# SJLeo/GCC

Measured on AMD Instinct MI355X. Metric: training images/sec at 256x256 (pix2pix GCC), higher is better.
Workload: dtype bf16; 1 GPU; Pix2Pix cityscapes 256x256 GCC distill+darts iteration (optimize_parameters + optimizer_netD_arch), student ngf32 / masked PatchGAN ndf128, teacher ngf64 / ndf128, filter_cfgs=None (no pretrained checkpoint to prune); batch_per_gpu=16, global_batch=16, image=256x256, parallelism=dp1, dropout=on (counter RNG; the oracle / golden iterations run --no_dropout)

## Files before the change

gcc_amd/csrc/conv_igemm.hip:

```cpp
#include <stdlib.h>
#include <mutex>
#include "common.hpp"
#include "igemm_common.hpp"

#ifndef GCC_IGEMM_ROT
#define GCC_IGEMM_ROT 0
#endif

namespace gcc_igemm {

#ifdef GCC_CLOCK_PROBE
__device__ unsigned long long g_clock_probe[4096][8];
#endif

template <int BP, int BC, bool UT, int NS = 2, bool EV = false>
__global__ __launch_bounds__((BP / 32) * 64) void igemm_kernel(const IgemmArgs<EV> p) {
    constexpr int EPI = EV ? 1 : 0;
#include "igemm_kernel_body.inc"
}

template <int BP, int BC, bool UT, int NS = 2>
__global__ __launch_bounds__((BP / 32) * 64) void igemm_ex_kernel(const IgemmExParams p) {
    constexpr int EPI = 2;
#include "igemm_kernel_body.inc"
// ... 375 lines not shown
    else if (Cout > 32) { t.BC = 64; t.ntiles = 1; }
    else if (Cout > 16) { t.BC = 32; t.ntiles = 1; }
    else { t.BC = 16; t.ntiles = 1; }
    if (batch == 1 && t.BC > 32) {
        const long mt = (long)((max_rows + 127) / 128) * phases;
        if (nk <= 64) {
            int bc = t.BC;
            while (bc > 32 && mt * cdiv(Cout, bc) < 256) bc >>= 1;
            if (mt * cdiv(Cout, bc) >= 256) { t.BC = bc; t.ntiles = cdiv(Cout, bc); }
        } else if (mt >= 8 && mt * cdiv(Cout, t.BC) < 128) {
            t.BC = 64; t.ntiles = cdiv(Cout, 64); t.max_slices = 8;
        }
    }
    const int g_big_tiles = plan_or(pl.tile_families, PLAN_TILE_FAMILIES) - 1, g_big_min = plan_or(pl.big_min, PLAN_BIG_MIN),
              g_big_nk = plan_or(pl.big_nk, PLAN_BIG_NK);
    if (g_big_tiles && batch == 1 && Cout >= 128 && nk >= g_big_nk) {
        const long m256 = (long)((max_rows + 255) / 256);
        if (g_big_tiles >= 2 && Cout % 256 == 0 && m256 * (Cout / 256) * phases >= g_big_min) {
            t.BP = 256; t.BC = 256; t.ntiles = Cout / 256;
            t.pair = (pl.pair == 1 && m256 * (Cout / 256) * phases < 192 && nk >= 48) ? 1 : 0;
        } else if (m256 * cdiv(Cout, 128) * phases >= g_big_min) {
            t.BP = 256; t.BC = 128; t.ntiles = cdiv(Cout, 128);
        }
    }
    t.mtiles = (int)((max_rows + t.BP - 1) / t.BP);
    return t;
}
constexpr size_t PAIR_FLAG_BYTES = 4096;
static size_t pair_workspace(size_t tiles) { return tiles > 512 ? ~(size_t)0 : PAIR_FLAG_BYTES + tiles * (size_t)(256 * 256 * 4); }
static int conv_nk(const gcc_conv_t* c, int dgrad) {
    const int taps_max = dgrad ? cdiv(c->KH, c->stride) * cdiv(c->KW, c->stride) : c->KH * c->KW;
    return cdiv(taps_max * ceil8(dgrad ? c->Co : c->Ci), BK);
}
static size_t conv_max_rows(const gcc_conv_t* c, int dgrad) {
    if (!dgrad) return (size_t)c->N * gcc_conv_out(c->H, c->KH, c->stride, c->pad) * gcc_conv_out(c->W, c->KW, c->stride, c->pad);
    return (size_t)c->N * cdiv(c->H, c->stride) * cdiv(c->W, c->stride);
}

int check_conv(const gcc_conv_t* c) {
    if (!c) return GCC_ERR_BAD_ARG;
    if (c->N <= 0 || c->H <= 0 || c->W <= 0 || c->Ci <= 0 || c->Co <= 0 || c->KH <= 0 || c->KW <= 0 ||
        c->stride <= 0 || c->pad < 0)
        return GCC_ERR_BAD_ARG;
    if ((c->ldx & 7) || (c->xoff & 7) || (c->ldy & 7) || (c->yoff & 7)) return GCC_ERR_BAD_ARG;
    if (c->ldx < c->xoff + ceil8(c->Ci) || c->ldy < c->yoff + ceil8(c->Co)) return GCC_ERR_BAD_ARG;
    if (gcc_conv_out(c->H, c->KH, c->stride, c->pad) <= 0 || gcc_conv_out(c->W, c->KW, c->stride, c->pad) <= 0)
        return GCC_ERR_BAD_ARG;
    return GCC_OK;
}

}
using namespace gcc_igemm;

struct HeadArgs {
    const float* partial; int ksplit, rows_max, Cpad;
    const float* bias; int act; float slope;
    bf16_t* dst; int ldd, doff;
    const bf16_t* dy; int lddy, dyoff;
    bf16_t* g;
    int N, H, W, Ho, Wo, KH, KW, stride, pad;
};
__global__ __launch_bounds__(256) void head_tapsum_kernel(const HeadArgs a) {
    const size_t total = (size_t)a.N * a.Ho * a.Wo;
    const int tap = threadIdx.x & 15;
    const int kh = tap / a.KW, kw = tap - kh * a.KW;
    for (size_t q0 = (size_t)blockIdx.x * 16; q0 < total; q0 += (size_t)gridDim.x * 16) {
        const size_t q = q0 + (threadIdx.x >> 4);
        float acc = 0.f;
        if (q < total && kh < a.KH) {
            const int ox = (int)(q % a.Wo);
            const size_t t = q / a.Wo;
            const int oy = (int)(t % a.Ho);
            const size_t n = t / a.Ho;
            const int iy = oy * a.stride + kh - a.pad, ix = ox * a.stride + kw - a.pad;
            if ((unsigned)iy < (unsigned)a.H && (unsigned)ix < (unsigned)a.W) {
                const size_t row = (n * a.H + iy) * (size_t)a.W + ix;
                for (int s = 0; s < a.ksplit; s++) acc += a.partial[((size_t)s * a.rows_max + row) * a.Cpad + tap];
            }
        }
#pragma unroll
        for (int o = 8; o > 0; o >>= 1) acc += __shfl_xor(acc, o, 16);
        if (tap == 0 && q < total) {
            float o[8] = {0, 0, 0, 0, 0, 0, 0, 0};
            o[0] = apply_act(acc + (a.bias ? a.bias[0] : 0.f), a.act, a.slope);
            *(i32x4*)(a.dst + q * a.ldd + a.doff) = pack8(o);
        }
    }
}
__global__ __launch_bounds__(256) void head_gather_kernel(const HeadArgs a) {
    const int taps = a.KH * a.KW;
    const size_t total = (size_t)a.N * a.H * a.W * taps;
    for (size_t q = (size_t)blockIdx.x * 256 + threadIdx.x; q < total; q += (size_t)gridDim.x * 256) {
        const int tap = (int)(q % taps);
        const size_t pix = q / taps;
        const int ix = (int)(pix % a.W);
        const size_t t = pix / a.W;
        const int iy = (int)(t % a.H);
        const size_t n = t / a.H;
        const int kh = tap / a.KW, kw = tap - kh * a.KW;
        const int ny = iy + a.pad - kh, nx = ix + a.pad - kw;
        float o[8] = {0, 0, 0, 0, 0, 0, 0, 0};
        if (ny >= 0 && nx >= 0 && ny % a.stride == 0 && nx % a.stride == 0) {
            const int oy = ny / a.stride, ox = nx / a.stride;
            if (oy < a.Ho && ox < a.Wo) o[0] = bf2f(a.dy[((n * a.Ho + oy) * (size_t)a.Wo + ox) * a.lddy + a.dyoff]);
        }
        *(i32x4*)(a.g + q * 8) = pack8(o);
// ... 429 lines not shown
        std::call_once(wide_once, [] {
            (void)hipFuncSetAttribute((const void*)thin_dgrad_wide_kernel, hipFuncAttributeMaxDynamicSharedMemorySize, 156 * 1024);
        });
        int wpi = 256 / c->N;
        if (wpi < 1) wpi = 1;
        if (wpi > a.Ho) wpi = a.Ho;
        const int rows_per_wg = cdiv(a.Ho, wpi);
        wpi = cdiv(a.Ho, rows_per_wg);
        hipLaunchKernelGGL(thin_dgrad_wide_kernel, dim3(c->N * wpi), dim3(THIN_WIDE_NT), lds, st, a, rows_per_wg, wpi);
        GCC_CHECK_LAUNCH();
        return GCC_OK;
    }
    const int ncc = a.Co8 > 32 ? 2 : 1;
    int wgs = cdiv(a.ntiles, 4);
    if (wgs > 768) wgs = 768;
    const dim3 grid(wgs, 2);
    if (ncc == 2) hipLaunchKernelGGL(thin_dgrad_k4s2_kernel<2>, grid, dim3(256), 0, st, a);
    else hipLaunchKernelGGL(thin_dgrad_k4s2_kernel<1>, grid, dim3(256), 0, st, a);
    GCC_CHECK_LAUNCH();
    return GCC_OK;
}

extern "C" int gcc_conv_y2_supported(const gcc_conv_t* c, int dgrad, const gcc_epilogue_t* ep) {
    if (check_conv(c) || dgrad || !ep || !thin_shape(c)) return 0;
    if (ep->stats_partial || ep->act == GCC_ACT_TANH || (ep->act == GCC_ACT_LRELU && (ep->slope < 0.f || ep->slope > 1.f))) return 0;
    if ((ep->ldy2 & 7) || (ep->y2off & 7)) return 0;
    if (ep->y2_mode == 1) return ep->act == GCC_ACT_LRELU || ep->act == GCC_ACT_NONE;
    if (ep->y2_mode == 2) return ep->y2_gate != nullptr;
    return 0;
}

int gcc_internal_thinout_fprop(const gcc_conv_t* c, const void* x, const void* w, void* y, const gcc_epilogue_t* ep, hipStream_t st);
int gcc_internal_thinout_dgrad(const gcc_conv_t* c, const void* dy, const void* wt, void* dx, const gcc_epilogue_t* ep, hipStream_t st);
int gcc_internal_ring3(const gcc_conv_t* c, int dgrad, const void* src, const void* w, void* dst, const gcc_epilogue_t* ep, hipStream_t st);
int gcc_internal_ring3_rows(const gcc_conv_t* c, int dgrad);
bool gcc_internal_ring3_routed(const gcc_conv_t* c, int dgrad, const gcc_epilogue_t* ep);

constexpr size_t FUSE_BN_PARTIAL_BYTES = (size_t)4096 * 1024;

int gcc_internal_igemm(const gcc_conv_t* c, int dgrad, const void* src, const void* w, void* dst, const gcc_epilogue_t* ep,
                       int batch, long src_bstride, long wgt_bstride, long dst_bstride, hipStream_t st) {
    GCC_ENTER();
    int rc = check_conv(c);
    if (rc) return rc;
    if (!src || !w || !dst) return GCC_ERR_BAD_ARG;
    const int Ho = gcc_conv_out(c->H, c->KH, c->stride, c->pad);
    const int Wo = gcc_conv_out(c->W, c->KW, c->stride, c->pad);
    if (batch == 1 && head_shape(c) && ep && ep->workspace && !ep->stats_partial && (((uintptr_t)ep->workspace) & 15) == 0) {
        const int taps = c->KH * c->KW;
        if (!dgrad) {
            int ks = 1;
            const size_t need = head_fprop_workspace(c, &ks);
            if (need <= ep->workspace_bytes) {
                IgemmParams q;
                q.src = (const bf16_t*)src; q.wgt = (const bf16_t*)w; q.dst = (bf16_t*)dst; q.bias = nullptr; q.stats = nullptr;
                q.act = GCC_ACT_NONE; q.slope = 0.f;
                q.N = c->N; q.KH = 1; q.KW = 1; q.stride = 1; q.pad = 0; q.dgrad = 0;
                q.Hs = c->H; q.Ws = c->W; q.lds_ = c->ldx; q.soff = c->xoff; q.Hd = c->H; q.Wd = c->W; q.ldd = c->ldy; q.doff = c->yoff;
                q.Ct = ceil8(c->Ci); q.Cout = taps; q.ldw = q.Ct;
                const size_t rows = head_rows(c);
                const size_t sb = rows * (size_t)q.lds_ * 2, wb = (size_t)taps * q.ldw * 2;
                if (sb < OOB && wb < OOB) {
                    q.src_bytes = (uint32_t)sb; q.wgt_bytes = (uint32_t)wb;
                    q.src_bstride = q.wgt_bstride = q.dst_bstride = 0;
                    q.ntiles = 1; q.mtiles_max = cdiv((int)rows, 128);
                    const int nk = cdiv(q.Ct, BK);
                    q.ksplit = ks; q.kper = cdiv(nk, ks); q.partial = (float*)ep->workspace; q.rows_max = (int)rows; q.Cpad = 16;
                    q.raw_partial = 1;
                    int rc2 = launch<128, 16>(q, 1, 1, st);
                    if (rc2) return rc2;
                    HeadArgs a = {};
                    a.partial = q.partial; a.ksplit = q.ksplit; a.rows_max = q.rows_max; a.Cpad = 16;
                    a.bias = ep->bias; a.act = ep->act; a.slope = ep->slope;
                    a.dst = (bf16_t*)dst; a.ldd = c->ldy; a.doff = c->yoff;
                    a.N = c->N; a.H = c->H; a.W = c->W; a.Ho = Ho; a.Wo = Wo; a.KH = c->KH; a.KW = c->KW; a.stride = c->stride; a.pad = c->pad;
                    const size_t outs = (size_t)c->N * Ho * Wo;
                    hipLaunchKernelGGL(head_tapsum_kernel, dim3((unsigned)(outs + 15 > 16 * 4096 ? 4096 : (outs + 15) / 16)), dim3(256), 0, st, a);
                    GCC_CHECK_LAUNCH();
                    return GCC_OK;
                }
            }
        }
    }
    if (batch == 1 && dgrad && thin_dgrad_shape(c) && !(ep && ep->stats_partial)) {
        const int rc2 = launch_thin_dgrad(c, src, w, dst, ep, st);
        if (rc2 >= 0) return rc2;
    }
    if (batch == 1) {
        const int rc3 = dgrad ? gcc_internal_thinout_dgrad(c, src, w, dst, ep, st) : gcc_internal_thinout_fprop(c, src, w, dst, ep, st);
        if (rc3 != GCC_ERR_UNSUPPORTED) return rc3;
        const int rc4 = gcc_internal_ring3(c, dgrad, src, w, dst, ep, st);
        if (rc4 != GCC_ERR_UNSUPPORTED) return rc4;
    }
    if (ep && ep->y2) {
        if (!gcc_conv_y2_supported(c, dgrad, ep)) return GCC_ERR_UNSUPPORTED;
    }
    if (batch == 1 && !dgrad && thin_shape(c) &&
        !(ep && (ep->stats_partial || ep->act == GCC_ACT_TANH || (ep->act == GCC_ACT_LRELU && (ep->slope < 0.f || ep->slope > 1.f))))) {
        const int rc2 = launch_thin(c, src, w, dst, ep, st);
        if (rc2 >= 0) return rc2;
    }
    if (ep && ep->y2) return GCC_ERR_UNSUPPORTED;
    IgemmParams p;
    p.src = (const bf16_t*)src; p.wgt = (const bf16_t*)w; p.dst = (bf16_t*)dst;
    p.bias = ep ? ep->bias : nullptr;
    p.stats = ep ? ep->stats_partial : nullptr;
    p.act = ep ? ep->act : GCC_ACT_NONE;
    p.slope = ep ? ep->slope : 0.f;
    p.N = c->N; p.KH = c->KH; p.KW = c->KW; p.stride = c->stride; p.pad = c->pad; p.dgrad = dgrad;
    size_t src_pix, max_rows;
    if (!dgrad) {
        p.Hs = c->H; p.Ws = c->W; p.lds_ = c->ldx; p.soff = c->xoff;
        p.Hd = Ho; p.Wd = Wo; p.ldd = c->ldy; p.doff = c->yoff;
        p.Ct = ceil8(c->Ci); p.Cout = c->Co;
        max_rows = (size_t)c->N * Ho * Wo;
    } else {
        p.Hs = Ho; p.Ws = Wo; p.lds_ = c->ldy; p.soff = c->yoff;
        p.Hd = c->H; p.Wd = c->W; p.ldd = c->ldx; p.doff = c->xoff;
        p.Ct = ceil8(c->Co); p.Cout = c->Ci;
        const int s = c->stride;
        max_rows = (size_t)c->N * cdiv(c->H, s) * cdiv(c->W, s);
    }
    src_pix = (size_t)p.N * p.Hs * p.Ws;
    p.ldw = c->KH * c->KW * p.Ct;
    const size_t sb = src_pix * (size_t)p.lds_ * 2, wb = (size_t)p.Cout * p.ldw * 2;
    const size_t db = (size_t)p.N * p.Hd * p.Wd * p.ldd * 2;
    if (sb >= OOB || wb >= OOB || db >= (size_t)1 << 32) return GCC_ERR_UNSUPPORTED;
    p.src_bytes = (uint32_t)sb; p.wgt_bytes = (uint32_t)wb;
    p.src_bstride = src_bstride; p.wgt_bstride = wgt_bstride; p.dst_bstride = dst_bstride;
    if (batch < 1 || (batch > 1 && p.stats)) return GCC_ERR_BAD_ARG;
    const int phases = dgrad ? c->stride * c->stride : 1;
    if (dgrad && (c->KH < c->stride || c->KW < c->stride)) return GCC_ERR_UNSUPPORTED;
    const TilePlan tp = select_tile(c->plan, max_rows, p.Cout, phases, conv_nk(c, dgrad), batch);
    const gcc_bn_t* bnf = (ep && ep->bn && p.stats && batch == 1) ? ep->bn : nullptr;
    const int rows_alloc = p.stats ? gcc_conv_stat_tiles(c, dgrad) : 0;
// ... 66 lines not shown
        tail_direct = make_tail(rows, p.ntiles, &fin_direct);
        if (tail_direct) p.fin = fin_direct;
    }
    if (tp.BP == 256) {
        rc = BC == 256 ? launch<256, 256>(p, phases, batch, st) : launch<256, 128>(p, phases, batch, st);
    } else {
        switch (BC) {
            case 128: rc = launch<128, 128>(p, phases, batch, st); break;
            case 64: rc = launch<128, 64>(p, phases, batch, st); break;
            case 32: rc = launch<128, 32>(p, phases, batch, st); break;
            default: rc = launch<128, 16>(p, phases, batch, st); break;
        }
    }
    if (rc) return rc;
    if (fold_stats) {
        FoldStatsArgs a;
        a.p = p; a.p.stats = stats_out;
        a.wpp = fold_wpp(max_rows, phases);
        a.rpw = (int)((max_rows + a.wpp - 1) / a.wpp);
        const int CH = ceil8(p.Cout) / 8;
        a.CHP = 1; a.sh = 0;
        while (a.CHP < CH) { a.CHP <<= 1; a.sh++; }
        TailFin fin;
        const bool tail = make_tail(a.wpp * phases, 1, &fin);
        a.p.fin = tail ? fin : TailFin{};
        hipLaunchKernelGGL(splitk_fold_stats_kernel, dim3(a.wpp, 1, phases), dim3(256), 0, st, a);
        GCC_CHECK_LAUNCH();
        return tail ? GCC_OK : finalize_after();
    }
    if (p.ksplit > 1 && stats_out && !p.pair) {
        const size_t pixels = (size_t)p.N * p.Hd * p.Wd;
        hipLaunchKernelGGL(channel_stats_kernel, dim3(ceil8(p.Cout) / 8), dim3(256), 0, st, p.dst, p.ldd, p.doff, p.Cout,
                           pixels, stats_out, rows_alloc);
        GCC_CHECK_LAUNCH();
        return finalize_after();
    }
    return tail_direct ? GCC_OK : finalize_after();
}

#ifdef GCC_CLOCK_PROBE
extern "C" int gcc_probe_read(unsigned long long* dst, int clear) {
    hipError_t e = hipMemcpyFromSymbol(dst, HIP_SYMBOL(gcc_igemm::g_clock_probe), sizeof(unsigned long long) * 4096 * 8);
    if (e == hipSuccess && clear) {
        void* sym = nullptr;
        if (hipGetSymbolAddress(&sym, HIP_SYMBOL(gcc_igemm::g_clock_probe)) == hipSuccess) e = hipMemset(sym, 0, sizeof(unsigned long long) * 4096 * 8);
    }
    return e == hipSuccess ? 0 : -1;
}
#endif

bool gcc_internal_thinout_routed(const gcc_conv_t* c, int dgrad, const gcc_epilogue_t* ep);
extern "C" int gcc_conv_route(const gcc_conv_t* c, int dgrad, const gcc_epilogue_t* ep) {
    if (check_conv(c)) return -1;
    if (gcc_internal_thinout_routed(c, dgrad, ep) && !(!dgrad && head_shape(c))) return 3;
    if (gcc_internal_ring3_routed(c, dgrad, ep) && !(!dgrad && head_shape(c)) && !(dgrad && thin_dgrad_shape(c) && !(ep && ep->stats_partial)))
        return 4;
    if (dgrad && thin_dgrad_shape(c) && !(ep && ep->stats_partial)) return 1;
    if (!dgrad && thin_shape(c) &&
        !(ep && (ep->stats_partial || ep->act == GCC_ACT_TANH || (ep->act == GCC_ACT_LRELU && (ep->slope < 0.f || ep->slope > 1.f)))))
        return 1;
    if (!dgrad && head_shape(c) && ep && ep->workspace && !ep->stats_partial && (((uintptr_t)ep->workspace) & 15) == 0 &&
        head_fprop_workspace(c, nullptr) <= ep->workspace_bytes)
        return 2;
    return 0;
}

namespace gcc_igemm {
struct FoldBnArgs {
    IgemmParams p;
    gcc_bn_t bn;
    int act, act2; float slope, drop_p; uint64_t seed;
    bf16_t* y; int ldy, yoff;
    bf16_t* y2; int ldy2, y2off;
    int phases;
};
template <int NT>
__global__ __launch_bounds__(NT) void splitk_bn_act_kernel(const FoldBnArgs a) {
    __shared__ double red[NT / 64][16];
    __shared__ float coef[16];
    const IgemmParams& p = a.p;
    const int c0 = blockIdx.x * 8;
    const int C = p.Cout;
    const size_t sstride = (size_t)p.rows_max * p.Cpad;
    double s[8], ss[8];
#pragma unroll
    for (int j = 0; j < 8; j++) s[j] = ss[j] = 0.0;
    for (int z = 0; z < a.phases; z++) {
        int py = 0, px = 0, Hg, Wg, ostr = 1;
        if (!p.dgrad) { Hg = p.Hd; Wg = p.Wd; }
        else {
            const int st = p.stride;
            py = z / st; px = z % st; ostr = st;
            Hg = (p.Hd - py + st - 1) / st; Wg = (p.Wd - px + st - 1) / st;
        }
        const int M = p.N * Hg * Wg;
        const float* base = p.partial + (size_t)z * p.ksplit * sstride;
        for (int m = threadIdx.x; m < M; m += NT) {
            float v[8] = {0, 0, 0, 0, 0, 0, 0, 0};
            const float* r0 = base + (size_t)m * p.Cpad + c0;
            int sl = 0;
            for (; sl + 4 <= p.ksplit; sl += 4) {
                f32x4 u[4], w[4];
#pragma unroll
                for (int q = 0; q < 4; q++) {
                    u[q] = *(const f32x4*)(r0 + (sl + q) * sstride);
                    w[q] = *(const f32x4*)(r0 + (sl + q) * sstride + 4);
// ... 456 lines not shown
```

gcc_amd/csrc/conv_wgrad.hip:

```cpp
#include <mutex>
#include <string.h>
#include "common.hpp"

namespace {

struct WgradParams {
    const bf16_t* x;
    const bf16_t* dy;
    float* out;
    int N, H, W, ldx, xoff, Cip, Ci;
    int Ho, Wo, ldy, yoff, Co;
    int KH, KW, stride, pad;
    int ncols;
    int M;
    int ksteps_per_split;
    int col_tiles, co_tiles;
    uint32_t x_bytes, dy_bytes;
    FastDiv dHW, dW, dCip, dKW;
    int batch;
    long x_bstride, dy_bstride;
    int direct;
    int accumulate;
    float* dw;
    int rowmode;
// ... 575 lines not shown
    const int per = cdiv(blocks, splits);
    *blocks_per_split = per;
    return cdiv(blocks, per);
}

int plan_splits(const gcc_conv_t* c, int batch, int* ksteps_per_split, bool* big_out = nullptr) {
    const int Ho = gcc_conv_out(c->H, c->KH, c->stride, c->pad), Wo = gcc_conv_out(c->W, c->KW, c->stride, c->pad);
    const long M = (long)c->N * Ho * Wo;
    const int ksteps = (int)((M + TP - 1) / TP);
    const int ncols = c->KH * c->KW * ceil8(c->Ci);
    constexpr int BIG_MIN_TILES = 8;
    const int tiles_big = cdiv(ncols, 256) * cdiv(c->Co, 256);
    bool big = batch == 1 && (c->Ci & 7) == 0 && c->Co >= 256 && ncols >= 256 && tiles_big >= BIG_MIN_TILES && ksteps >= 64;
    int splits;
    if (big) {
        const int target = plan_or(c->plan.wgrad_wgs_big, PLAN_WGRAD_WGS_BIG);
        splits = tiles_big >= (target * 25) / 32 ? 1 : cdiv(target, tiles_big);
        const int max_splits = ksteps / 16 > 0 ? ksteps / 16 : 1;
        if (splits > max_splits) splits = max_splits;
    } else {
        const int tiles = cdiv(ncols, 128) * cdiv(c->Co, 128) * batch;
        const int target = plan_or(c->plan.wgrad_wgs, PLAN_WGRAD_WGS);
        splits = tiles >= (target * 3) / 8 ? 1 : cdiv(target, tiles);
        const int max_splits = ksteps / 8 > 0 ? ksteps / 8 : 1;
        if (splits > max_splits) splits = max_splits;
    }
    if (splits < 1) splits = 1;
    const int per = cdiv(ksteps, splits);
    splits = cdiv(ksteps, per);
    *ksteps_per_split = per;
    if (big_out) *big_out = big;
    return splits;
}

}

size_t gcc_internal_wgrad_workspace(const gcc_conv_t* c, int batch) {
    if (!c || c->Ci <= 0 || c->Co <= 0 || batch < 1) return 0;
    int per, tper;
    int splits = plan_splits(c, batch, &per);
    const int tsplits = ts_plan(c, batch, &tper);
    if (tsplits > splits) splits = tsplits;
    return (size_t)splits * batch * c->Co * c->KH * c->KW * ceil8(c->Ci) * sizeof(float);
}

size_t gcc_internal_head_gather_bytes(const gcc_conv_t* c);
int gcc_internal_head_gather(const gcc_conv_t* c, const void* dy, void* g, hipStream_t st);
static size_t al256(size_t v) { return (v + 255) & ~(size_t)255; }
static gcc_conv_t head_conv1x1(const gcc_conv_t* c) {
    const int taps = c->KH * c->KW;
    gcc_conv_t c1 = {c->N, c->H, c->W, c->Ci, taps * 8, 1, 1, 1, 0, c->ldx, c->xoff, taps * 8, 0};
    return c1;
}
static size_t head_wgrad_workspace(const gcc_conv_t* c) {
    const size_t g = gcc_internal_head_gather_bytes(c);
    if (!g) return 0;
    const gcc_conv_t c1 = head_conv1x1(c);
    return al256(g) + al256((size_t)c1.Co * ceil8(c->Ci) * sizeof(float)) + gcc_internal_wgrad_workspace(&c1, 1);
}
__global__ void head_rows_fold_kernel(const float* __restrict__ big, float* __restrict__ dw, int taps, int Cip, int accumulate) {
    const int n = taps * Cip;
    for (int i = blockIdx.x * blockDim.x + threadIdx.x; i < n; i += gridDim.x * blockDim.x) {
        const int t = i / Cip, cc = i - t * Cip;
        const float v = big[(size_t)(t * 8) * Cip + cc];
        dw[i] = accumulate ? dw[i] + v : v;
    }
}

size_t gcc_internal_thinout_wgrad_workspace(const gcc_conv_t* c);
int gcc_internal_thinout_wgrad(const gcc_conv_t* c, const void* x, const void* dy, float* dw, int accumulate, void* ws, size_t ws_bytes,
                               hipStream_t st);

extern "C" size_t gcc_conv_wgrad_workspace(const gcc_conv_t* c) {
    const size_t h = c ? head_wgrad_workspace(c) : 0;
    if (h) return h;
    const size_t t = c ? gcc_internal_thinout_wgrad_workspace(c) : 0, g = gcc_internal_wgrad_workspace(c, 1);
    return t > g ? t : g;
}

int gcc_internal_wgrad(const gcc_conv_t* c, const void* x, const void* dy, float* dw, int accumulate, void* ws,
                       size_t ws_bytes, int batch, long x_bstride, long dy_bstride, hipStream_t st, int rows_l,
                       int cols_l, int row_split, int col_split) {
    GCC_ENTER();
    if (!c || !x || !dy || !dw || !ws) return GCC_ERR_BAD_ARG;
    if (c->N <= 0 || c->H <= 0 || c->W <= 0 || c->Ci <= 0 || c->Co <= 0 || c->KH <= 0 || c->KW <= 0 ||
        c->stride <= 0 || c->pad < 0)
        return GCC_ERR_BAD_ARG;
    if ((c->ldx & 7) || (c->xoff & 7) || (c->ldy & 7) || (c->yoff & 7)) return GCC_ERR_BAD_ARG;
    const int Ho = gcc_conv_out(c->H, c->KH, c->stride, c->pad), Wo = gcc_conv_out(c->W, c->KW, c->stride, c->pad);
    if (Ho <= 0 || Wo <= 0) return GCC_ERR_BAD_ARG;
    if (batch < 1 || ws_bytes < gcc_internal_wgrad_workspace(c, batch)) return GCC_ERR_WORKSPACE;
    WgradParams p;
    p.x = (const bf16_t*)x; p.dy = (const bf16_t*)dy; p.out = (float*)ws;
    p.N = c->N; p.H = c->H; p.W = c->W; p.ldx = c->ldx; p.xoff = c->xoff; p.Ci = c->Ci; p.Cip = ceil8(c->Ci);
    p.Ho = Ho; p.Wo = Wo; p.ldy = c->ldy; p.yoff = c->yoff; p.Co = c->Co;
    p.KH = c->KH; p.KW = c->KW; p.stride = c->stride; p.pad = c->pad;
    p.ncols = c->KH * c->KW * p.Cip;
    const size_t M = (size_t)c->N * Ho * Wo;
    const size_t xb = (size_t)c->N * c->H * c->W * c->ldx * 2, yb = M * c->ldy * 2;
    if (xb >= OOB || yb >= OOB || M >= (1u << 30)) return GCC_ERR_UNSUPPORTED;
    p.M = (int)M; p.x_bytes = (uint32_t)xb; p.dy_bytes = (uint32_t)yb;
    bool big = false;
    const int splits = plan_splits(c, batch, &p.ksteps_per_split, &big);
    p.batch = batch; p.x_bstride = x_bstride; p.dy_bstride = dy_bstride;
    const bool seg = rows_l > 0;
    const bool regular = !seg && (c->Ci & 7) == 0 && (((uintptr_t)dw) & 15) == 0;
    big = big && regular;
// ... 48 lines not shown
    std::call_once(attr_once, [] {
        hipFuncSetAttribute((const void*)wgrad_kernel<false, false>, hipFuncAttributeMaxDynamicSharedMemorySize, WCfg<false>::LDS_BYTES);
        hipFuncSetAttribute((const void*)wgrad_kernel<true, false>, hipFuncAttributeMaxDynamicSharedMemorySize, WCfg<true>::LDS_BYTES);
        hipFuncSetAttribute((const void*)wgrad_kernel<false, true>, hipFuncAttributeMaxDynamicSharedMemorySize, WCfg<false>::LDS_BYTES);
        hipFuncSetAttribute((const void*)wgrad_kernel<true, true>, hipFuncAttributeMaxDynamicSharedMemorySize, WCfg<true>::LDS_BYTES);
    });
    const dim3 grid(p.col_tiles * p.co_tiles, batch, splits);
    if (big && p.rowmode)
        hipLaunchKernelGGL((wgrad_kernel<true, true>), grid, dim3(WCfg<true>::NT), WCfg<true>::LDS_BYTES, st, p);
    else if (big)
        hipLaunchKernelGGL((wgrad_kernel<true, false>), grid, dim3(WCfg<true>::NT), WCfg<true>::LDS_BYTES, st, p);
    else if (p.rowmode)
        hipLaunchKernelGGL((wgrad_kernel<false, true>), grid, dim3(WCfg<false>::NT), WCfg<false>::LDS_BYTES, st, p);
    else
        hipLaunchKernelGGL((wgrad_kernel<false, false>), grid, dim3(WCfg<false>::NT), WCfg<false>::LDS_BYTES, st, p);
    GCC_CHECK_LAUNCH();
    if (p.direct) return GCC_OK;
    const size_t total = (size_t)batch * c->Co * c->KH * c->KW * c->Ci;
    if (regular) {
        const size_t n4 = total / 4;
        if (splits <= 8) {
            int blocks = (int)((n4 + 255) / 256);
            if (blocks > 8192) blocks = 8192;
            hipLaunchKernelGGL(wgrad_reduce_flat_kernel, dim3(blocks), dim3(256), 0, st, (const float*)ws, dw, splits, n4,
                               accumulate);
        } else {
            int blocks = (int)((n4 + 63) / 64);
            if (blocks > 4096) blocks = 4096;
            hipLaunchKernelGGL(wgrad_reduce_vec_kernel, dim3(blocks), dim3(256), 0, st, (const float*)ws, dw, splits, n4,
                               accumulate);
        }
    } else {
        const size_t outs = seg ? (size_t)rows_l * c->KH * c->KW * cols_l : total;
        const bool deep = splits >= 32;
        int blocks = (int)((outs + (deep ? 15 : 63)) / (deep ? 16 : 64));
        if (blocks > 4096) blocks = 4096;
        const int rows = seg ? rows_l : batch * c->Co, cols = seg ? cols_l : c->Ci, cop = seg ? c->Co : batch * c->Co;
        const int rsp = seg ? row_split : 0, csp = seg ? col_split : 0;
        if (deep)
            hipLaunchKernelGGL((wgrad_reduce_kernel<16, 16>), dim3(blocks), dim3(256), 0, st, (const float*)ws, dw, splits, rows,
                               c->KH * c->KW, cols, p.Cip, accumulate, cop, rsp, csp);
        else
            hipLaunchKernelGGL((wgrad_reduce_kernel<64, 4>), dim3(blocks), dim3(256), 0, st, (const float*)ws, dw, splits, rows,
                               c->KH * c->KW, cols, p.Cip, accumulate, cop, rsp, csp);
    }
    GCC_CHECK_LAUNCH();
    return GCC_OK;
}

extern "C" int gcc_conv_wgrad(const gcc_conv_t* c, const void* x, const void* dy, float* dw, int accumulate,
                              void* ws, size_t ws_bytes, gcc_stream_t stream) {
    GCC_ENTER();
    const size_t hw = c ? head_wgrad_workspace(c) : 0;
    if (hw && ws && ws_bytes >= hw && x && dy && dw && (c->Ci & 7) == 0) {
        hipStream_t st = (hipStream_t)stream;
        char* base = (char*)ws;
        const gcc_conv_t c1 = head_conv1x1(c);
        const size_t gbytes = al256(gcc_internal_head_gather_bytes(c));
        const size_t bbytes = al256((size_t)c1.Co * c->Ci * sizeof(float));
        int rc = gcc_internal_head_gather(c, dy, base, st);
        if (rc) return rc;
        float* big = (float*)(base + gbytes);
        rc = gcc_internal_wgrad(&c1, x, base, big, 0, base + gbytes + bbytes, ws_bytes - gbytes - bbytes, 1, 0, 0, st, 0, 0, 0, 0);
        if (rc) return rc;
        const int taps = c->KH * c->KW;
        hipLaunchKernelGGL(head_rows_fold_kernel, dim3((taps * c->Ci + 255) / 256), dim3(256), 0, st, (const float*)big, dw, taps, c->Ci,
                           accumulate);
        GCC_CHECK_LAUNCH();
        return GCC_OK;
    }
    if (c && x && dy && dw && ws && (((uintptr_t)dw) & 3) == 0) {
        const int rc = gcc_internal_thinout_wgrad(c, x, dy, dw, accumulate, ws, ws_bytes, (hipStream_t)stream);
        if (rc != GCC_ERR_UNSUPPORTED) return rc;
    }
    return gcc_internal_wgrad(c, x, dy, dw, accumulate, ws, ws_bytes, 1, 0, 0, (hipStream_t)stream, 0, 0, 0, 0);
}

extern "C" int gcc_conv_wgrad_seg(const gcc_conv_t* c, const void* x, const void* dy, float* dw, int rows, int cols,
                                  int row_split, int col_split, int accumulate, void* ws, size_t ws_bytes,
                                  gcc_stream_t stream) {
    GCC_ENTER();
    if (!c || rows <= 0 || cols <= 0) return GCC_ERR_BAD_ARG;
    if (c->Co != seg_phys_size(rows, row_split) || c->Ci != seg_phys_size(cols, col_split)) return GCC_ERR_BAD_ARG;
    return gcc_internal_wgrad(c, x, dy, dw, accumulate, ws, ws_bytes, 1, 0, 0, (hipStream_t)stream, rows, cols, row_split,
                              col_split);
}

namespace {
struct GroupPlan {
    int n, total_wgs;
    int per[GROUP_MAX], splits[GROUP_MAX], tiles[GROUP_MAX], order[GROUP_MAX];
    size_t slab_off[GROUP_MAX], ws_bytes;
};
int group_cus() {
    static const int v = [] {
        int dev = 0, n = 0;
        if (hipGetDevice(&dev) != hipSuccess || hipDeviceGetAttribute(&n, hipDeviceAttributeMultiprocessorCount, dev) != hipSuccess || n <= 0) {
            (void)hipGetLastError();
            n = 256;
        }
        return n;
    }();
    return v;
}
bool group_item_ok(const gcc_wgrad_item_t* it) {
    const gcc_conv_t* c = &it->c;
    if (c->N <= 0 || c->H <= 0 || c->W <= 0 || c->Ci <= 0 || c->Co <= 0 || c->KH <= 0 || c->KW <= 0 || c->stride <= 0 || c->pad < 0) return false;
// ... 126 lines not shown
```

gcc_amd/ops.py:

```python
import ctypes as C
import os
import threading

import torch

from . import _lib
from ._lib import ACT_LRELU, ACT_NONE, ACT_RELU, ACT_TANH, check

_ws_cache = {}


class _Profile:

    def __init__(self):
        self.active = False
        self.spans_only = False
        self.records = []
        self.streaming = os.environ.get('GCC_PROFILE_STREAMING') == '1'

    def start(self, steps=None):
        self.records = []
        self.spans = []
        self.tag = None
        self.active = True
# ... 74 lines not shown
            t['spans'] = t.get('spans', 0) + 1
        self.spans = []
        if os.environ.get('GCC_PROFILE_SHAPES') == '1':
            import sys
            for (kind, shape, tag), (fl, sec, n) in sorted(shapes.items(), key=lambda kv: -kv[1][1])[:int(os.environ.get('GCC_PROFILE_TOP', '200'))]:
                print('%-14s %-44s %-14s n=%4d  total %7.3f ms  avg %7.1f us  %7.1f TFLOP/s' % (
                    kind, shape, tag, n, sec * 1e3, sec / n * 1e6, fl / sec / 1e12), file=sys.stderr)
        if not agg:
            return None
        dom = max(agg, key=lambda k: agg[k][1])
        out = None
        per = {}
        for kind, (fl, sec, n) in agg.items():
            per[kind] = {'launches': n, 'avg_us': round(1e6 * sec / n, 2), 'tflops': round(fl / sec / 1e12, 2),
                         'time_s': round(sec, 4), 'gflop': round(fl / 1e9, 3)}
            if kind == dom:
                out = {'bound': 'mfma', 'kernel': kind, 'achieved': round(fl / sec / 1e12, 2), 'peak': peak / 1e12,
                       'unit': 'TFLOP/s', 'frac': round(fl / sec / peak, 4), 'traffic': None, 'launches': n,
                       'steps_bracketed': getattr(self, 'steps_seen', None),
                       'avg_launch_us': round(1e6 * sec / n, 2),
                       'algorithmic_gflop_per_launch': round(fl / n / 1e9, 3),
                       'algorithmic_bytes_per_launch': round(alg_bytes.get(kind, 0.0) / n)}
        out['per_kernel'] = per
        if roof_n:
            out['conv_roofline'] = {'layers': roof_n, 'bound_ms': round(roof_s * 1e3, 3), 'measured_ms': round(roof_meas_s * 1e3, 3),
                                    'frac': round(roof_s / roof_meas_s, 4),
                                    'definition': 'sum over the conv launches of one iteration of max(FLOP / 2.5 PFLOP/s, '
                                                  'minimum operand bytes / 8 TB/s) over the sum of their measured durations'}
        return out


class _Span:
    def __init__(self, prof, name):
        self.prof, self.name = prof, name

    def __enter__(self):
        if self.prof.active or self.prof.spans_only:
            self.prev = self.prof.tag
            self.prof.tag = self.name
            self.e0 = torch.cuda.Event(enable_timing=True)
            self.e0.record()
        return self

    def __exit__(self, *exc):
        if getattr(self, 'e0', None) is not None:
            e1 = torch.cuda.Event(enable_timing=True)
            e1.record()
            self.prof.spans.append((self.name, self.e0, e1))
            self.prof.tag = self.prev
        return False


PROFILE = _Profile()
_ROUTE_KIND = {0: 'igemm_kernel (conv fprop/dgrad)', 1: 'thin_fprop / thin_dgrad (image layers)', 2: 'head route (igemm 128x16 + tap sum)',
               3: 'thinout_fprop / thinout_dgrad (wide filters, <= 3 output channels)',
               4: 'ring3_kernel (3 x 3 stride 1, <= 64 channels both sides)', -1: 'igemm_kernel (conv fprop/dgrad)'}


def lib():
    return _lib.load()


_dev_index = None


def set_device_index(idx):
    global _dev_index
    _dev_index = idx


_RAW_STREAM = getattr(torch._C, '_cuda_getCurrentRawStream', None)
_SET_STREAM = getattr(torch._C, '_cuda_setStream', None)
if os.environ.get('GCC_PUBLIC_STREAM_API') == '1':
    _RAW_STREAM = _SET_STREAM = None


def _set_current(s):
    global _SET_STREAM
    if _SET_STREAM is not None:
        try:
            _SET_STREAM(stream_id=s.stream_id, device_index=s.device_index, device_type=s.device_type)
            return
        except (TypeError, AttributeError):
            _SET_STREAM = None
    torch.cuda.set_stream(s)


def stream():
    global _dev_index, _RAW_STREAM
    if _dev_index is None:
        _dev_index = torch.cuda.current_device()
    if _RAW_STREAM is not None:
        try:
            return _RAW_STREAM(_dev_index)
        except (TypeError, AttributeError):
            _RAW_STREAM = None
    return torch.cuda.current_stream(_dev_index).cuda_stream


_stream_objs = {}


def current_stream():
    raw = stream()
    s = _stream_objs.get(raw)
    if s is None:
        s = _stream_objs[raw] = torch.cuda.current_stream()
# ... 1199 lines not shown
```

Baseline: 1067 images/s.

## Add dedicated fused kernels for 4x4 single-channel PatchGAN head conv

Adds a new conv_head.hip with specialized fprop, dgrad and wgrad kernels for the Co=1, 4x4, stride-1, pad-1 discriminator head. Fprop fuses the per-tap MFMA GEMM and the tap sum within one block using LDS, replacing a split-K igemm launch followed by a tap-sum kernel. Dgrad and wgrad stage dy tiles in LDS and do direct FMA accumulation, with per-block partials folded by a small reduction kernel, replacing the gather plus 1x1 wgrad path. This costs large LDS use and high register pressure (16x8 accumulators), and reduction order changes slightly.

Result: no change. 1071 images/s, median of 6 (+0.4%).

```diff
diff --git a/gcc_amd/csrc/conv_head.hip b/gcc_amd/csrc/conv_head.hip
--- /dev/null
+++ b/gcc_amd/csrc/conv_head.hip
@@ -0,0 +1,371 @@
+#include "common.hpp"
+#include <mutex>
+
+namespace {
+
+constexpr int SLICE = 256;
+constexpr size_t HEAD_OOB = (size_t)1 << 31;
+
+constexpr int FWD_NT = 1024, FWD_WAVES = FWD_NT / 64, FWD_TB = 16, FWD_TP = FWD_TB + 3, FWD_U = 16;
+constexpr int FWD_T_FLOATS = FWD_TP * FWD_TP * 16;
+struct HeadFwdArgs {
+    const bf16_t* x; const bf16_t* w; bf16_t* y; const float* bias;
+    int act; float slope;
+    int N, H, W, Ho, Wo, Ci, ldx, xoff, ldy, yoff;
+    int nty, ntx, nks;
+};
+__global__ __launch_bounds__(FWD_NT) void head_fwd_kernel(const HeadFwdArgs a) {
+    extern __shared__ __attribute__((aligned(16))) char head_lds[];
+    i32x4* wl = (i32x4*)head_lds;
+    float* T = (float*)(head_lds + (size_t)a.nks * 1024);
+    const int tid = threadIdx.x, lane = tid & 63, wave = tid >> 6;
+    const int bid = xcd_remap(blockIdx.x, gridDim.x);
+    const int tx = bid % a.ntx, ty = (bid / a.ntx) % a.nty, n = bid / (a.ntx * a.nty);
+    const int oy0 = ty * a.Ho / a.nty, oy1 = (ty + 1) * a.Ho / a.nty, ox0 = tx * a.Wo / a.ntx, ox1 = (tx + 1) * a.Wo / a.ntx;
+    const int th = oy1 - oy0, tw = ox1 - ox0, ph = th + 3, pw = tw + 3, npix = ph * pw;
+    const int nchunks = a.Ci >> 3;
+    for (int e = tid; e < a.nks * 64; e += FWD_NT) {
+        const int c8 = (e >> 6) * 4 + ((e & 63) >> 4), t = e & 15;
+        i32x4 v = {0, 0, 0, 0};
+        if (c8 < nchunks) v = *(const i32x4*)(a.w + (size_t)t * a.Ci + c8 * 8);
+        wl[e] = v;
+    }
+    const int groups = (npix + 15) >> 4;
+    const int ksplit = (groups * 2 <= FWD_WAVES && a.nks >= 2) ? 2 : 1;
+    const int kper = (a.nks + ksplit - 1) / ksplit;
+    __syncthreads();
+    const int r = lane & 15, g = lane >> 4;
+    for (int item = wave; item < groups * ksplit; item += FWD_WAVES) {
+        const int grp = item % groups, sp = item / groups;
+        const int q = grp * 16 + r;
+        const int py = q / pw, px = q - py * pw;
+        const int iy = oy0 - 1 + py, ix = ox0 - 1 + px;
+        const bool valid = q < npix && (unsigned)iy < (unsigned)a.H && (unsigned)ix < (unsigned)a.W;
+        const bf16_t* xp = a.x + (valid ? (((size_t)n * a.H + iy) * a.W + ix) * a.ldx + a.xoff : 0);
+        const int k0 = sp * kper, k1 = min(k0 + kper, a.nks);
+        f32x4 acc = {0.f, 0.f, 0.f, 0.f};
+        for (int ks = k0; ks < k1; ks += FWD_U) {
+            i32x4 xv[FWD_U];
+#pragma unroll
+            for (int u = 0; u < FWD_U; u++) {
+                const int c8 = (ks + u) * 4 + g;
+                xv[u] = i32x4{0, 0, 0, 0};
+                if (valid && ks + u < k1 && c8 < nchunks) xv[u] = *(const i32x4*)(xp + c8 * 8);
+            }
+#pragma unroll
+            for (int u = 0; u < FWD_U; u++) {
+                const i32x4 wv = wl[min(ks + u, a.nks - 1) * 64 + lane];
+                acc = __builtin_amdgcn_mfma_f32_16x16x32_bf16(__builtin_bit_cast(bf16x8, xv[u]), __builtin_bit_cast(bf16x8, wv), acc, 0, 0, 0);
+            }
+        }
+#pragma unroll
+        for (int i = 0; i < 4; i++) {
+            const int qo = grp * 16 + g * 4 + i;
+            if (qo < npix) T[((size_t)sp * npix + qo) * 16 + r] = acc[i];
+        }
+    }
+    __syncthreads();
+    const int tap = tid & 15, kh = tap >> 2, kw = tap & 3;
+    const int nout = th * tw;
+    for (int o0 = 0; o0 < nout; o0 += FWD_NT / 16) {
+        const int o = o0 + (tid >> 4);
+        float v = 0.f;
+        int oy = 0, ox = 0;
+        if (o < nout) {
+            oy = o / tw; ox = o - oy * tw;
+            const int p = (oy + kh) * pw + ox + kw;
+            v = T[(size_t)p * 16 + tap];
+            if (ksplit == 2) v += T[((size_t)npix + p) * 16 + tap];
+        }
+#pragma unroll
+        for (int s = 8; s > 0; s >>= 1) v += __shfl_xor(v, s, 16);
+        if (tap == 0 && o < nout) {
+            float out[8] = {0, 0, 0, 0, 0, 0, 0, 0};
+            out[0] = apply_act(v + (a.bias ? a.bias[0] : 0.f), a.act, a.slope);
+            *(i32x4*)(a.y + (((size_t)n * a.Ho + oy0 + oy) * a.Wo + ox0 + ox) * a.ldy + a.yoff) = pack8(out);
+        }
+    }
+}
+
+struct HeadGradArgs {
+    const bf16_t* x; const bf16_t* dy; const bf16_t* wt; bf16_t* dx; float* part;
+    int N, H, W, Ho, Wo, Ci, ldx, xoff, ldy, yoff;
+    int P, rows_total, RC, Cs;
+    FastDiv dW;
+};
+__device__ __forceinline__ void stage_dy(const HeadGradArgs& a, float* tile, int jbase, int nrows, int tid, int nt) {
+    const int tw = a.W + 3, per = 4 * tw;
+    for (int e = tid; e < nrows * per; e += nt) {
+        const int j = e / per, rem = e - j * per, r4 = rem / tw, col = rem - r4 * tw;
+        const int rr = blockIdx.x + (jbase + j) * a.P;
+        const int n = rr / a.H, iy = rr - n * a.H;
+        const int oy = iy - 2 + r4, ox = col - 2;
+        float v = 0.f;
+        if ((unsigned)oy < (unsigned)a.Ho && (unsigned)ox < (unsigned)a.Wo)
+            v = bf2f(a.dy[(((size_t)n * a.Ho + oy) * a.Wo + ox) * a.ldy + a.yoff]);
+        tile[e] = v;
+    }
+}
+__device__ __forceinline__ void read_dy(const float* tile, int tw, int j, int ix, float* d) {
+#pragma unroll
+    for (int kh = 0; kh < 4; kh++)
+#pragma unroll
+        for (int kw = 0; kw < 4; kw++) d[kh * 4 + kw] = tile[(j * 4 + 3 - kh) * tw + ix + 3 - kw];
+}
+__device__ __forceinline__ int rows_of(const HeadGradArgs& a) { return (a.rows_total - (int)blockIdx.x + a.P - 1) / a.P; }
+
+constexpr int DG_NT = 512, DG_WPAD = SLICE + 4;
+__global__ __launch_bounds__(DG_NT) void head_dgrad_kernel(const HeadGradArgs a) {
+    extern __shared__ __attribute__((aligned(16))) char head_lds[];
+    float* ws = (float*)head_lds;
+    float* tile = ws + 16 * DG_WPAD;
+    const int tid = threadIdx.x, lane = tid & 63, hl = lane & 31, slot = tid >> 5;
+    const int cbase = blockIdx.y * SLICE, c0 = cbase + hl * 8;
+    const bool active = c0 < a.Ci;
+    for (int e = tid; e < SLICE * 16; e += DG_NT) {
+        const int cl = e >> 4, tap = e & 15;
+        ws[tap * DG_WPAD + cl] = cbase + cl < a.Ci ? bf2f(a.wt[((size_t)(cbase + cl) * 16 + tap) * 8]) : 0.f;
+    }
+    __syncthreads();
+    float wv[16][8];
+#pragma unroll
+    for (int t = 0; t < 16; t++) {
+        const f32x4 lo = *(const f32x4*)(ws + t * DG_WPAD + hl * 8), hi = *(const f32x4*)(ws + t * DG_WPAD + hl * 8 + 4);
+#pragma unroll
+        for (int j = 0; j < 4; j++) { wv[t][j] = lo[j]; wv[t][4 + j] = hi[j]; }
+    }
+    const int tw = a.W + 3, nrows = rows_of(a);
+    for (int jbase = 0; jbase < nrows; jbase += a.RC) {
+        const int nr = min(a.RC, nrows - jbase);
+        __syncthreads();
+        stage_dy(a, tile, jbase, nr, tid, DG_NT);
+        __syncthreads();
+        for (int it = slot; it < nr * a.W; it += DG_NT / 32) {
+            const int j = fdiv(it, a.dW), ix = it - j * a.W;
+            float d[16];
+            read_dy(tile, tw, j, ix, d);
+            float acc[8] = {0, 0, 0, 0, 0, 0, 0, 0};
+#pragma unroll
+            for (int t = 0; t < 16; t++)
+#pragma unroll
+                for (int c = 0; c < 8; c++) acc[c] = fmaf(d[t], wv[t][c], acc[c]);
+            const size_t rr = (size_t)blockIdx.x + (size_t)(jbase + j) * a.P;
+            if (active) *(i32x4*)(a.dx + (rr * a.W + ix) * a.ldx + a.xoff + c0) = pack8(acc);
+        }
+    }
+}
+
+constexpr int WG_NT = 512, WG_WAVES = WG_NT / 64, WG_U = 8;
+constexpr int WG_RED_FLOATS = WG_WAVES * 16 * SLICE;
+__global__ __launch_bounds__(WG_NT) void head_wgrad_kernel(const HeadGradArgs a) {
+    extern __shared__ __attribute__((aligned(16))) char head_lds[];
+    float* tile = (float*)head_lds;
+    const int tid = threadIdx.x, lane = tid & 63, hl = lane & 31, slot = tid >> 5, wave = tid >> 6;
+    const int cbase = blockIdx.y * SLICE, c0 = cbase + hl * 8;
+    const bool active = c0 < a.Ci;
+    float acc[16][8];
+#pragma unroll
+    for (int t = 0; t < 16; t++)
+#pragma unroll
+        for (int c = 0; c < 8; c++) acc[t][c] = 0.f;
+    const int tw = a.W + 3, nrows = rows_of(a);
+    for (int jbase = 0; jbase < nrows; jbase += a.RC) {
+        const int nr = min(a.RC, nrows - jbase);
+        __syncthreads();
+        stage_dy(a, tile, jbase, nr, tid, WG_NT);
+        __syncthreads();
+        const int items = nr * a.W;
+        for (int it0 = slot; it0 < items; it0 += WG_U * (WG_NT / 32)) {
+            i32x4 xv[WG_U];
+#pragma unroll
+            for (int u = 0; u < WG_U; u++) {
+                const int it = it0 + u * (WG_NT / 32);
+                xv[u] = i32x4{0, 0, 0, 0};
+                if (active && it < items) {
+                    const int j = fdiv(it, a.dW), ix = it - j * a.W;
+                    const size_t rr = (size_t)blockIdx.x + (size_t)(jbase + j) * a.P;
+                    xv[u] = *(const i32x4*)(a.x + (rr * a.W + ix) * a.ldx + a.xoff + c0);
+                }
+            }
+#pragma unroll
+            for (int u = 0; u < WG_U; u++) {
+                const int it = it0 + u * (WG_NT / 32);
+                if (it < items) {
+                    const int j = fdiv(it, a.dW), ix = it - j * a.W;
+                    float d[16], xf[8];
+                    read_dy(tile, tw, j, ix, d);
+                    unpack8(xv[u], xf);
+#pragma unroll
+                    for (int t = 0; t < 16; t++)
+#pragma unroll
+                        for (int c = 0; c < 8; c++) acc[t][c] = fmaf(d[t], xf[c], acc[t][c]);
+                }
+            }
+        }
+    }
+    float* red = (float*)head_lds;
+    float* mine = red + ((size_t)wave * 16) * SLICE + hl * 8;
+    __syncthreads();
+    if (lane < 32) {
+#pragma unroll
+        for (int t = 0; t < 16; t++) {
+            *(f32x4*)(mine + t * SLICE) = f32x4{acc[t][0], acc[t][1], acc[t][2], acc[t][3]};
+            *(f32x4*)(mine + t * SLICE + 4) = f32x4{acc[t][4], acc[t][5], acc[t][6], acc[t][7]};
+        }
+    }
+    __syncthreads();
+    if (lane >= 32) {
+#pragma unroll
+        for (int t = 0; t < 16; t++) {
+            const f32x4 lo = *(const f32x4*)(mine + t * SLICE), hi = *(const f32x4*)(mine + t * SLICE + 4);
+            *(f32x4*)(mine + t * SLICE) = f32x4{lo[0] + acc[t][0], lo[1] + acc[t][1], lo[2] + acc[t][2], lo[3] + acc[t][3]};
+            *(f32x4*)(mine + t * SLICE + 4) = f32x4{hi[0] + acc[t][4], hi[1] + acc[t][5], hi[2] + acc[t][6], hi[3] + acc[t][7]};
+        }
+    }
+    __syncthreads();
+    for (int e = tid; e < 16 * SLICE / 4; e += WG_NT) {
+        f32x4 sum = *(const f32x4*)(red + (size_t)e * 4);
+#pragma unroll
+        for (int w = 1; w < WG_WAVES; w++) {
+            const f32x4 v = *(const f32x4*)(red + (size_t)w * 16 * SLICE + (size_t)e * 4);
+#pragma unroll
+            for (int c = 0; c < 4; c++) sum[c] += v[c];
+        }
+        const int t = e / (SLICE / 4), c4 = e - t * (SLICE / 4);
+        *(f32x4*)(a.part + ((size_t)blockIdx.x * 16 + t) * a.Cs + cbase + c4 * 4) = sum;
+    }
+}
+constexpr int FOLD_U = 16;
+__global__ __launch_bounds__(256) void head_wgrad_fold_kernel(const float* __restrict__ part, float* __restrict__ dw, int P, int Cs, int Ci,
+                                                              int accumulate) {
+    __shared__ float sh[4][64];
+    const int o = threadIdx.x & 63, q = threadIdx.x >> 6;
+    const int i = blockIdx.x * 64 + o;
+    const bool ok = i < 16 * Ci;
+    const int per = (P + 3) / 4, p0 = q * per, p1 = min(P, p0 + per);
+    float s = 0.f;
+    if (ok) {
+        const int t = i / Ci, c = i - t * Ci;
+        const float* src = part + (size_t)t * Cs + c;
+        for (int p = p0; p < p1; p += FOLD_U) {
+            float v[FOLD_U];
+#pragma unroll
+            for (int u = 0; u < FOLD_U; u++) v[u] = p + u < p1 ? src[(size_t)(p + u) * 16 * Cs] : 0.f;
+#pragma unroll
+            for (int u = 0; u < FOLD_U; u++) s += v[u];
+        }
+    }
+    sh[q][o] = s;
+    __syncthreads();
+    if (q == 0 && ok) {
+        const float r = ((sh[0][o] + sh[1][o]) + sh[2][o]) + sh[3][o];
+        dw[i] = accumulate ? dw[i] + r : r;
+    }
+}
+
+int head_cus() {
+    static const int v = [] {
+        int dev = 0, n = 0;
+        if (hipGetDevice(&dev) != hipSuccess || hipDeviceGetAttribute(&n, hipDeviceAttributeMultiprocessorCount, dev) != hipSuccess || n <= 0) {
+            (void)hipGetLastError();
+            n = 256;
+        }
+        return n;
+    }();
+    return v;
+}
+constexpr size_t HEAD_LDS_MAX = (size_t)128 << 10;
+constexpr int TILE_FLOATS_MAX = 8192;
+bool head_attrs() {
+    static std::once_flag once;
+    static bool ok = false;
+    std::call_once(once, [] {
+        ok = hipFuncSetAttribute((const void*)head_fwd_kernel, hipFuncAttributeMaxDynamicSharedMemorySize, (int)HEAD_LDS_MAX) == hipSuccess &&
+             hipFuncSetAttribute((const void*)head_dgrad_kernel, hipFuncAttributeMaxDynamicSharedMemorySize, (int)HEAD_LDS_MAX) == hipSuccess &&
+             hipFuncSetAttribute((const void*)head_wgrad_kernel, hipFuncAttributeMaxDynamicSharedMemorySize, (int)HEAD_LDS_MAX) == hipSuccess;
+    });
+    return ok;
+}
+size_t fwd_lds(const gcc_conv_t* c) { return (size_t)cdiv(c->Ci, 32) * 1024 + (size_t)FWD_T_FLOATS * sizeof(float); }
+struct GradPlan { int slices, P, RC, rows_total; };
+GradPlan grad_plan(const gcc_conv_t* c) {
+    GradPlan g;
+    g.slices = cdiv(c->Ci, SLICE);
+    g.rows_total = c->N * c->H;
+    g.P = head_cus() / g.slices;
+    if (g.P < 1) g.P = 1;
+    if (g.P > g.rows_total) g.P = g.rows_total;
+    const int rows = cdiv(g.rows_total, g.P), cap = TILE_FLOATS_MAX / (4 * (c->W + 3));
+    g.RC = rows < cap ? rows : cap;
+    return g;
+}
+void fill_grad(HeadGradArgs& a, const gcc_conv_t* c, const GradPlan& g) {
+    a.N = c->N; a.H = c->H; a.W = c->W; a.Ho = c->H - 1; a.Wo = c->W - 1; a.Ci = c->Ci;
+    a.ldx = c->ldx; a.xoff = c->xoff; a.ldy = c->ldy; a.yoff = c->yoff;
+    a.P = g.P; a.rows_total = g.rows_total; a.RC = g.RC; a.Cs = g.slices * SLICE; a.dW = make_fastdiv(c->W);
+}
+
+}
+
+bool gcc_internal_head_k4(const gcc_conv_t* c) {
+    if (!(c->Co == 1 && c->KH == 4 && c->KW == 4 && c->stride == 1 && c->pad == 1 && (c->Ci & 7) == 0 && c->Ci >= 256)) return false;
+    if (c->H < 2 || c->W < 2 || 4 * (c->W + 3) > TILE_FLOATS_MAX || fwd_lds(c) > HEAD_LDS_MAX) return false;
+    const size_t px = (size_t)c->N * c->H * c->W;
+    return px * c->ldx * 2 < HEAD_OOB && px * c->ldy * 2 < HEAD_OOB;
+}
+
+int gcc_internal_head_fprop(const gcc_conv_t* c, const void* x, const void* w, void* y, const gcc_epilogue_t* ep, hipStream_t st) {
+    if (!gcc_internal_head_k4(c) || (ep && (ep->stats_partial || ep->y2))) return GCC_ERR_UNSUPPORTED;
+    if ((((uintptr_t)x | (uintptr_t)w | (uintptr_t)y) & 15) || !head_attrs()) return GCC_ERR_UNSUPPORTED;
+    HeadFwdArgs a = {};
+    a.x = (const bf16_t*)x; a.w = (const bf16_t*)w; a.y = (bf16_t*)y;
+    a.bias = ep ? ep->bias : nullptr; a.act = ep ? ep->act : GCC_ACT_NONE; a.slope = ep ? ep->slope : 0.f;
+    a.N = c->N; a.H = c->H; a.W = c->W; a.Ho = c->H - 1; a.Wo = c->W - 1; a.Ci = c->Ci;
+    a.ldx = c->ldx; a.xoff = c->xoff; a.ldy = c->ldy; a.yoff = c->yoff; a.nks = cdiv(c->Ci, 32);
+    static const int edges[] = {16, 12, 10, 8, 6, 5, 4};
+    for (int tb : edges) {
+        a.nty = cdiv(a.Ho, tb); a.ntx = cdiv(a.Wo, tb);
+        if ((long)a.N * a.nty * a.ntx >= head_cus()) break;
+    }
+    hipLaunchKernelGGL(head_fwd_kernel, dim3((unsigned)(a.N * a.nty * a.ntx)), dim3(FWD_NT), fwd_lds(c), st, a);
+    GCC_CHECK_LAUNCH();
+    return GCC_OK;
+}
+
+int gcc_internal_head_dgrad(const gcc_conv_t* c, const void* dy, const void* wt, void* dx, const gcc_epilogue_t* ep, hipStream_t st) {
+    if (!gcc_internal_head_k4(c)) return GCC_ERR_UNSUPPORTED;
+    if (ep && (ep->bias || ep->act != GCC_ACT_NONE || ep->stats_partial || ep->y2)) return GCC_ERR_UNSUPPORTED;
+    if ((((uintptr_t)dx) & 15) || (((uintptr_t)wt | (uintptr_t)dy) & 1) || !head_attrs()) return GCC_ERR_UNSUPPORTED;
+    const GradPlan g = grad_plan(c);
+    HeadGradArgs a = {};
+    a.dy = (const bf16_t*)dy; a.wt = (const bf16_t*)wt; a.dx = (bf16_t*)dx;
+    fill_grad(a, c, g);
+    const size_t lds = ((size_t)16 * DG_WPAD + (size_t)g.RC * 4 * (c->W + 3)) * sizeof(float);
+    hipLaunchKernelGGL(head_dgrad_kernel, dim3(g.P, g.slices), dim3(DG_NT), lds, st, a);
+    GCC_CHECK_LAUNCH();
+    return GCC_OK;
+}
+
+size_t gcc_internal_head_wgrad_bytes(const gcc_conv_t* c) {
+    if (!c || c->N <= 0 || c->H <= 0 || c->W <= 0 || c->Ci <= 0 || c->ldx < c->xoff + c->Ci || c->ldy < c->yoff + 8) return 0;
+    if ((c->ldx & 7) || (c->xoff & 7) || (c->ldy & 7) || (c->yoff & 7) || !gcc_internal_head_k4(c)) return 0;
+    const GradPlan g = grad_plan(c);
+    return (size_t)g.P * 16 * g.slices * SLICE * sizeof(float);
+}
+int gcc_internal_head_wgrad(const gcc_conv_t* c, const void* x, const void* dy, float* dw, int accumulate, void* ws, size_t ws_bytes,
+                            hipStream_t st) {
+    const size_t need = gcc_internal_head_wgrad_bytes(c);
+    if (!need || (((uintptr_t)x | (uintptr_t)ws) & 15) || (((uintptr_t)dw) & 3) || !head_attrs()) return GCC_ERR_UNSUPPORTED;
+    if (ws_bytes < need) return GCC_ERR_WORKSPACE;
+    const GradPlan g = grad_plan(c);
+    HeadGradArgs a = {};
+    a.x = (const bf16_t*)x; a.dy = (const bf16_t*)dy; a.part = (float*)ws;
+    fill_grad(a, c, g);
+    const size_t tile = (size_t)g.RC * 4 * (c->W + 3) * sizeof(float), red = (size_t)WG_RED_FLOATS * sizeof(float);
+    hipLaunchKernelGGL(head_wgrad_kernel, dim3(g.P, g.slices), dim3(WG_NT), tile > red ? tile : red, st, a);
+    GCC_CHECK_LAUNCH();
+    hipLaunchKernelGGL(head_wgrad_fold_kernel, dim3(cdiv(16 * c->Ci, 64)), dim3(256), 0, st, (const float*)ws, dw, g.P, g.slices * SLICE,
+                       c->Ci, accumulate);
+    GCC_CHECK_LAUNCH();
+    return GCC_OK;
+}
diff --git a/gcc_amd/csrc/conv_igemm.hip b/gcc_amd/csrc/conv_igemm.hip
--- a/gcc_amd/csrc/conv_igemm.hip
+++ b/gcc_amd/csrc/conv_igemm.hip
@@ -451,6 +451,9 @@
 }
 using namespace gcc_igemm;
 
+bool gcc_internal_head_k4(const gcc_conv_t* c);
+int gcc_internal_head_fprop(const gcc_conv_t* c, const void* x, const void* w, void* y, const gcc_epilogue_t* ep, hipStream_t st);
+int gcc_internal_head_dgrad(const gcc_conv_t* c, const void* dy, const void* wt, void* dx, const gcc_epilogue_t* ep, hipStream_t st);
 struct HeadArgs {
     const float* partial; int ksplit, rows_max, Cpad;
     const float* bias; int act; float slope;
@@ -986,6 +989,8 @@
             int ks = 1;
             const size_t need = head_fprop_workspace(c, &ks);
             if (need <= ep->workspace_bytes) {
+                const int rch = gcc_internal_head_fprop(c, src, w, dst, ep, st);
+                if (rch != GCC_ERR_UNSUPPORTED) return rch;
                 IgemmParams q;
                 q.src = (const bf16_t*)src; q.wgt = (const bf16_t*)w; q.dst = (bf16_t*)dst; q.bias = nullptr; q.stats = nullptr;
                 q.act = GCC_ACT_NONE; q.slope = 0.f;
@@ -1015,6 +1020,10 @@
                 }
             }
         }
+    }
+    if (batch == 1 && dgrad && head_shape(c)) {
+        const int rch = gcc_internal_head_dgrad(c, src, w, dst, ep, st);
+        if (rch != GCC_ERR_UNSUPPORTED) return rch;
     }
     if (batch == 1 && dgrad && thin_dgrad_shape(c) && !(ep && ep->stats_partial)) {
         const int rc2 = launch_thin_dgrad(c, src, w, dst, ep, st);
@@ -1187,6 +1196,8 @@
 bool gcc_internal_thinout_routed(const gcc_conv_t* c, int dgrad, const gcc_epilogue_t* ep);
 extern "C" int gcc_conv_route(const gcc_conv_t* c, int dgrad, const gcc_epilogue_t* ep) {
     if (check_conv(c)) return -1;
+    if (dgrad && head_shape(c) && gcc_internal_head_k4(c) && !(ep && (ep->bias || ep->act != GCC_ACT_NONE || ep->stats_partial || ep->y2)))
+        return 2;
     if (gcc_internal_thinout_routed(c, dgrad, ep) && !(!dgrad && head_shape(c))) return 3;
     if (gcc_internal_ring3_routed(c, dgrad, ep) && !(!dgrad && head_shape(c)) && !(dgrad && thin_dgrad_shape(c) && !(ep && ep->stats_partial)))
         return 4;
diff --git a/gcc_amd/csrc/conv_wgrad.hip b/gcc_amd/csrc/conv_wgrad.hip
--- a/gcc_amd/csrc/conv_wgrad.hip
+++ b/gcc_amd/csrc/conv_wgrad.hip
@@ -651,7 +651,11 @@
     gcc_conv_t c1 = {c->N, c->H, c->W, c->Ci, taps * 8, 1, 1, 1, 0, c->ldx, c->xoff, taps * 8, 0};
     return c1;
 }
+size_t gcc_internal_head_wgrad_bytes(const gcc_conv_t* c);
+int gcc_internal_head_wgrad(const gcc_conv_t* c, const void* x, const void* dy, float* dw, int accumulate, void* ws, size_t ws_bytes,
+                            hipStream_t st);
 static size_t head_wgrad_workspace(const gcc_conv_t* c) {
+    if (const size_t k4 = gcc_internal_head_wgrad_bytes(c)) return k4;
     const size_t g = gcc_internal_head_gather_bytes(c);
     if (!g) return 0;
     const gcc_conv_t c1 = head_conv1x1(c);
@@ -806,7 +810,10 @@
                               void* ws, size_t ws_bytes, gcc_stream_t stream) {
     GCC_ENTER();
     const size_t hw = c ? head_wgrad_workspace(c) : 0;
-    if (hw && ws && ws_bytes >= hw && x && dy && dw && (c->Ci & 7) == 0) {
+    if (hw && ws && ws_bytes >= hw && x && dy && dw && gcc_internal_head_wgrad_bytes(c)) {
+        const int rch = gcc_internal_head_wgrad(c, x, dy, dw, accumulate, ws, ws_bytes, (hipStream_t)stream);
+        if (rch != GCC_ERR_UNSUPPORTED) return rch;
+    } else if (hw && ws && ws_bytes >= hw && x && dy && dw && (c->Ci & 7) == 0) {
         hipStream_t st = (hipStream_t)stream;
         char* base = (char*)ws;
         const gcc_conv_t c1 = head_conv1x1(c);
diff --git a/gcc_amd/ops.py b/gcc_amd/ops.py
--- a/gcc_amd/ops.py
+++ b/gcc_amd/ops.py
@@ -150,7 +150,7 @@
 
 
 PROFILE = _Profile()
-_ROUTE_KIND = {0: 'igemm_kernel (conv fprop/dgrad)', 1: 'thin_fprop / thin_dgrad (image layers)', 2: 'head route (igemm 128x16 + tap sum)',
+_ROUTE_KIND = {0: 'igemm_kernel (conv fprop/dgrad)', 1: 'thin_fprop / thin_dgrad (image layers)', 2: 'head route (conv_head.hip / igemm 128x16 + tap sum)',
                3: 'thinout_fprop / thinout_dgrad (wide filters, <= 3 output channels)',
                4: 'ring3_kernel (3 x 3 stride 1, <= 64 channels both sides)', -1: 'igemm_kernel (conv fprop/dgrad)'}
 
```
